# peach-xiao/EMRT

Hardware: AMD Instinct MI355X
Metric: training tiles/sec at 256x256 (higher is better)
Workload: dtype bf16; 1 GPU; EMRT ResNet50, Potsdam 256x256, 6 classes, batch 8 per GPU, fwd+bwd+SGD step (BASELINE configs[1]), bf16; global_batch=8, parallelism=dp1, hipgraph=True

## Files before the change

emrt_amd/csrc/common.hpp:

```cpp
#pragma once
#include <hip/hip_runtime.h>
#include <stdint.h>
#include <stdio.h>
#include <string.h>
#include "drop_hash.hpp"
#include "../../include/emrt_hip.h"

#define EMRT_F32 0
#define EMRT_BF16 1
#define EMRT_F16 2

namespace emrt {

extern thread_local char g_err[512];
inline int fail(const char* fn, const char* msg) {
  snprintf(g_err, sizeof(g_err), "%s: %s", fn, msg);
  return -1;
}
inline int check_launch(const char* fn) {
  hipError_t e = hipGetLastError();
  if (e != hipSuccess) {
    snprintf(g_err, sizeof(g_err), "%s: launch failed: %s", fn, hipGetErrorString(e));
    return -2;
  }
// ... 10 lines not shown
  int thin_cblk;
  int thin_blocks;
  int thin_ch;
  int no_thin_bwd;
  int igemm64_nst;
  int wgrad_nst;
  int pair_max;
  int msda_fwd_global;
  int msda_bwd_global;
  int msda_lds_min_pairs;
  int msda_bwd_dref_lds;
  int msda_band_halo;
  int msda_scatter_qsplit;
  int msda_scatter_cuts;
  int msda_fwd_chunks;
  int msda_fwd_threads;
  int msda_fwd_probe;
  int bn_block_kb;
  int bn_slice_c;
  int bn_operand_blocks;
  int ln_bwd_rows;
  int ln_bwd_max_blocks;
  int ln_bwd_threads;
  int ln_atomic;
  int gn_group_blocks;
  int gn_stat_rows;
  int gn_bwd_stat_rows;
  int gn_apply_rows;
  int igemm8p_probe;
  int igemm8p_cmajor;
  int igemm8p_min_blocks;
  int wgrad8p_min_steps;
  int wgrad8p_slab;
  int wgrad8p_xcd;
  int wgrad8p_force;
  int no_ksplit128;
  int wgrad_no_overwrite;
  int no_s2_dgrad;
  int wgroup_blocks;
  int wgroup_min_steps;
  int wgroup_max;
  int wgroup8;
  int wgroup8_blocks;
  int wgroup8_min_work;
  int msda_scatter_merge;
  int msda_scatter_mfma;
  int msda_mf_bands;
  int sgd_nt;
  int mha_bwd_split;
  int mha_valu;
  int no_bna;
  int memcpy_kernel;
  int xk;
};
extern Tuning g_tune;

struct Scratch {
  void* ptr; size_t bytes; void* stream;
  unsigned* tick;
  float* xk_part;
};
constexpr size_t SCRATCH_TICK_BYTES = 65536;
constexpr int SCRATCH_TICKS = (int)(SCRATCH_TICK_BYTES / 4);
constexpr size_t SCRATCH_XK_BYTES = 8u << 20;
extern Scratch g_scratch;

struct bf16_t {
  unsigned short v;
};
struct f16_t {
  unsigned short v;
};

__device__ __forceinline__ float to_f32(float x) { return x; }
__device__ __forceinline__ float to_f32(bf16_t x) { return __uint_as_float(((uint32_t)x.v) << 16); }
__device__ __forceinline__ float to_f32(f16_t x) { return (float)__builtin_bit_cast(_Float16, x.v); }
__device__ __forceinline__ float bf16_bits_to_f32(uint32_t lo16) { return __uint_as_float(lo16 << 16); }
__device__ __forceinline__ float f16_bits_to_f32(uint32_t lo16) { return (float)__builtin_bit_cast(_Float16, (unsigned short)lo16); }

template <class T>
__device__ __forceinline__ T from_f32(float f);
template <>
__device__ __forceinline__ float from_f32<float>(float f) {
  return f;
}
template <>
__device__ __forceinline__ bf16_t from_f32<bf16_t>(float f) {
  __bf16 b = (__bf16)f;
  bf16_t r;
  r.v = __builtin_bit_cast(unsigned short, b);
  return r;
}
template <>
__device__ __forceinline__ f16_t from_f32<f16_t>(float f) {
  f16_t r;
  r.v = __builtin_bit_cast(unsigned short, (_Float16)f);
  return r;
}
typedef __attribute__((ext_vector_type(2))) _Float16 emrt_half2_t;
typedef __attribute__((ext_vector_type(2))) float emrt_float2_t;
__device__ __forceinline__ uint32_t pack_f16x2(float lo, float hi) {
  emrt_half2_t h = __builtin_convertvector((emrt_float2_t){lo, hi}, emrt_half2_t);
  return __builtin_bit_cast(uint32_t, h);
}
__device__ __forceinline__ void unpack_f16x2(uint32_t w, float& lo, float& hi) {
  const emrt_half2_t h = __builtin_bit_cast(emrt_half2_t, w);
// ... 223 lines not shown
```

emrt_amd/csrc/conv.hip:

```cpp
#include "common.hpp"
#include "bn_operand.hpp"
#include <stdlib.h>
#include <type_traits>

using namespace emrt;

typedef __attribute__((ext_vector_type(8))) __bf16 bf16x8_t;
typedef __attribute__((ext_vector_type(4))) short short4_t;
typedef __attribute__((ext_vector_type(16))) float f32x16_t;

struct ConvArgs {
  const void* in = nullptr;
  const void* w = nullptr;
  void* out = nullptr;
  const float* bias = nullptr;
  const float* scale = nullptr;
  const void* res = nullptr;
  int N = 0, H = 0, W = 0, C = 0, ldin = 0;
  long long in_bs = 0;
  int OH = 0, OW = 0, OC = 0, ldout = 0;
  long long out_bs = 0;
  int ldres = 0;
  long long res_bs = 0;
  int KH = 0, KW = 0, stride = 0, pad = 0;
// ... 617 lines not shown
    }
  }
  if (p.stats) {
#pragma unroll
    for (int j = 0; j < TN; ++j) {
      const float s2 = st_s[j] + __shfl_xor(st_s[j], 32, 64);
      const float q2 = st_q[j] + __shfl_xor(st_q[j], 32, 64);
      const int n = bn * BN + (wc * TN + j) * 32 + frow;
      if (fh == 0 && n < p.OC) {
        double* rep = p.stats + (long long)(bm & 7) * 2 * p.OC;
        atomicAdd(rep + n, (double)s2);
        atomicAdd(rep + p.OC + n, (double)q2);
      }
    }
  }
}

template <class T, int TM, int TN, int WR, int WC, int MODE, bool VEC, int NST, int G>
__global__ __launch_bounds__(256 * G, (TM * TN == 1 && G == 1) ? 4 : 1) void igemm_kernel(ConvArgs p) {
  extern __shared__ __attribute__((aligned(16))) unsigned char smem_all[];
  igemm_body<T, TM, TN, WR, WC, MODE, VEC, NST, G>(p, (int)blockIdx.x, (int)gridDim.x, smem_all);
}

template <class T, int MODE>
__global__ __launch_bounds__(256, 4) void igemm_xk_kernel(ConvArgs p) {
  extern __shared__ __attribute__((aligned(16))) unsigned char smem_all[];
  igemm_body<T, 1, 1, 2, 2, MODE, true, 3, 1, false, true>(p, (int)blockIdx.x, (int)gridDim.x, smem_all);
}

template <class T>
__global__ __launch_bounds__(256, 4) void igemm_drop_kernel(ConvArgs p) {
  extern __shared__ __attribute__((aligned(16))) unsigned char smem_all[];
  igemm_body<T, 1, 1, 2, 2, 0, true, 3, 1, false, false, true>(p, (int)blockIdx.x, (int)gridDim.x, smem_all);
}

template <class T>
__global__ __launch_bounds__(256, 4) void igemm_s2_kernel(ConvArgs p) {
  extern __shared__ __attribute__((aligned(16))) unsigned char smem_all[];
  igemm_body<T, 1, 1, 2, 2, 1, true, 3, 1, true>(p, (int)blockIdx.x, (int)gridDim.x, smem_all);
}

template <class T, int G>
__global__ __launch_bounds__(256 * G, G == 1 ? 4 : 1) void igemm_bna_kernel(ConvArgs p) {
  extern __shared__ __attribute__((aligned(16))) unsigned char smem_all[];
  igemm_body<T, 1, 1, 2, 2, 0, true, (G == 2 ? 6 : 2), G, false, false, false, true>(p, (int)blockIdx.x, (int)gridDim.x, smem_all);
}
template <class T>
__global__ __launch_bounds__(256, 4) void igemm_xk_bna_kernel(ConvArgs p) {
  extern __shared__ __attribute__((aligned(16))) unsigned char smem_all[];
  igemm_body<T, 1, 1, 2, 2, 0, true, 2, 1, false, true, false, true>(p, (int)blockIdx.x, (int)gridDim.x, smem_all);
}

#include "igemm8p.hpp"

struct WgradArgs {
  const void* x = nullptr;
  const void* dy = nullptr;
  float* dw = nullptr;
  int N = 0, H = 0, W = 0, C = 0, ldx = 0;
  long long x_bs = 0;
  int OH = 0, OW = 0, OC = 0, lddy = 0;
  long long dy_bs = 0;
  int KH = 0, KW = 0, stride = 0, pad = 0;
  int dil = 1;
  int tiles_per_split = 0;
  float* dbias = nullptr;
  int overwrite = 0;
};

template <class T>
struct WgradCfg;
template <>
struct WgradCfg<bf16_t> {
  static constexpr int CPR = 16, RPP = 16, BKM = 64, PITCH = 320;
};
template <>
struct WgradCfg<float> {
  static constexpr int CPR = 32, RPP = 8, BKM = 32, PITCH = 528;
};

template <class T, bool VEC, int G, int NSTW = 2>
__device__ __forceinline__ void wgrad_body(const WgradArgs& p, const int block_x, const int block_y, const int block_z, unsigned char* smem_all) {
  using Cfg = WgradCfg<T>;
  constexpr int EPC = 16 / (int)sizeof(T);
  constexpr int CPR = Cfg::CPR, RPP = Cfg::RPP, BKM = Cfg::BKM, PITCH = Cfg::PITCH;
  constexpr int NST = VEC ? NSTW : 1;
  constexpr int STAGE_BYTES = 2 * BKM * PITCH;

  const int grp = G == 1 ? 0 : (int)threadIdx.x >> 8;
  unsigned char* smem = smem_all + grp * 2 * STAGE_BYTES;
  const int tid = threadIdx.x & 255, lane = tid & 63, wave = tid >> 6;
  const int wr = wave >> 1, wc = wave & 1;
  const int K = p.KH * p.KW * p.C;
  const int oc0 = block_y * 128, k0 = block_x * 128;
  const __amdgpu_buffer_rsrc_t rs_x = __builtin_amdgcn_make_buffer_rsrc((void*)p.x, 0, (int)BUF_RANGE, 0x00020000);
  const __amdgpu_buffer_rsrc_t rs_dy = __builtin_amdgcn_make_buffer_rsrc((void*)p.dy, 0, (int)BUF_RANGE, 0x00020000);

  const int col = tid % CPR, prow = tid / CPR;
  const int kq = k0 + col * EPC;
  const int tap = kq < K ? kq / p.C : 0;
  const int cq = kq - tap * p.C;
  const int kh = tap / p.KW, kw = tap - kh * p.KW;
  const int ocp = oc0 + col * EPC;
  const unsigned q_bad = kq < K ? 0u : BUF_OOB;
  const unsigned p_bad = ocp < p.OC ? 0u : BUF_OOB;
  int e_c[EPC], e_kh[EPC], e_kw[EPC];
// ... 305 lines not shown
  constexpr int BK = 8 * (16 / (int)sizeof(T));
  return (a.KH * a.KW * a.C + BK - 1) / BK;
}

template <class T>
static bool igemm_s2_ok(const ConvArgs& a) {
  constexpr int EPC = 16 / (int)sizeof(T);
  constexpr int BK = 8 * EPC;
  const long long M = (long long)a.N * a.OH * a.OW;
  if (a.KH * a.KW == 1 && g_tune.no_s2_dgrad != -1) return false;
  if (g_tune.no_s2_dgrad == 1 || a.stride != 2 || a.dil != 1 || a.C % BK != 0 || (a.OH & 1) || (a.OW & 1) || (M % 4) || ((M / 4) % 64) || a.OC <= 32 || a.OC % 8) return false;
  if (a.out_f32 || a.bias || a.scale) return false;
  auto al = [](const void* q) { return ((uintptr_t)q) % 16 == 0; };
  if (!al(a.out) || (a.res && !al(a.res)) || (a.mask_y && !al(a.mask_y)) || (a.stat_x && !al(a.stat_x))) return false;
  if (a.ldout % EPC || a.out_bs % EPC || (a.res && (a.ldres % EPC || a.res_bs % EPC)) || (a.mask_y && (a.ldy % EPC || a.y_bs % EPC)) ||
      (a.stat_x && (a.ldsx % EPC || a.sx_bs % EPC))) return false;
  return true;
}

template <class T>
static int igemm_xk_copies(const ConvArgs& a, hipStream_t st, int want) {
  constexpr int EPC = 16 / (int)sizeof(T);
  if (sizeof(T) != 2 || g_tune.xk < 0 || !g_scratch.xk_part || !g_scratch.tick || g_scratch.stream != (void*)st) return 0;
  if (a.OC <= 32 || a.OC % 8 || a.out_f32) return 0;
  auto al = [](const void* q) { return ((uintptr_t)q) % 16 == 0; };
  if (!al(a.out) || (a.res && !al(a.res)) || (a.mask_y && !al(a.mask_y)) || (a.stat_x && !al(a.stat_x))) return 0;
  if (a.ldout % EPC || a.out_bs % EPC || (a.res && (a.ldres % EPC || a.res_bs % EPC)) || (a.mask_y && (a.ldy % EPC || a.y_bs % EPC)) ||
      (a.stat_x && (a.ldsx % EPC || a.sx_bs % EPC))) return 0;
  const long long nb = conv_blocks(a, 64, 64);
  const int nkt = conv_k_tiles<T>(a);
  int S = want;
  if (S <= 0) {
    if (!((nb <= 64 && nkt >= 36) || (nb <= 128 && nkt >= 128))) return 0;
    S = 4;
  }
  if (S > nkt) S = nkt;
  if (S >= 2) {
    const int per = (nkt + S - 1) / S;
    S = (nkt + per - 1) / per;
  }
  if (S < 2 || nb > SCRATCH_TICKS || (size_t)nb * (size_t)S * 64 * 64 * 4 > SCRATCH_XK_BYTES) return 0;
  return S;
}

template <class T, int MODE>
static int launch_igemm_xk(const ConvArgs& a0, hipStream_t st, int S) {
  ConvArgs a = a0;
  const long long nb = conv_blocks(a, 64, 64);
  a.xk_S = S; a.xk_part = g_scratch.xk_part; a.xk_tick = g_scratch.tick;
  hipLaunchKernelGGL((igemm_xk_kernel<T, MODE>), dim3((unsigned)(nb * S)), dim3(256), (size_t)2 * 128 * 144, st, a);
  return check_launch("emrt_conv2d");
}


template <class T>
static bool conv_takes_128(const ConvArgs& a) {
  return a.OC > 64 && conv_k_tiles<T>(a) >= 16 && conv_blocks(a, 128, 128) >= 256;
}

enum ConvKind {
  CONV_NONE,
  CONV_DROP,
  CONV_S2,
  CONV_128x64,
  CONV_256x32,
  CONV_XK,
  CONV_8P,
  CONV_128,
  CONV_64
};
struct ConvPlan {
  ConvKind kind;
  int n;
  bool forced;
};

template <class T, int MODE, bool VEC>
static ConvPlan conv_plan(const ConvArgs& a, hipStream_t st) {
  constexpr bool VEC2 = VEC && sizeof(T) == 2;
  if (a.drop_seed) {
    constexpr int EPC = 16 / (int)sizeof(T);
    const bool vec_out = ((uintptr_t)a.out) % 16 == 0 && a.ldout % EPC == 0 && a.out_bs % EPC == 0 && a.OC % 8 == 0 && !a.out_f32 && !a.res && !a.mask_y;
    return {MODE == 0 && VEC && vec_out ? CONV_DROP : CONV_NONE, 1, false};
  }
  if (MODE == 1 && VEC && !g_tune.conv_tile && igemm_s2_ok<T>(a)) return {CONV_S2, 1, false};
  switch (g_tune.conv_tile) {
    case 1: return {CONV_64, 1, true};
    case 2: return {CONV_128x64, 1, true};
    case 3: return {CONV_128, 1, true};
    case 4: return {CONV_256x32, 1, true};
    case 5: if (VEC) return {CONV_64, 2, true}; break;
    case 6: if (VEC) return {CONV_64, 4, true}; break;
    case 7: if (VEC2 && igemm8p_ok<T>(a)) return {CONV_8P, 1, true}; break;
    case 8: if (VEC2) return {CONV_128, 2, true}; break;
    default: break;
  }
  if (a.OC <= 32) return {CONV_256x32, 1, false};
  if (VEC2 && !g_tune.conv_tile) {
    const int S = igemm_xk_copies<T>(a, st, g_tune.xk > 0 ? g_tune.xk : 0);
    if (S >= 2) return {CONV_XK, S, false};
  }
  if (VEC2) {
    const long long nb256 = conv_blocks(a, 256, 256);
    const int nkt64 = a.KH * a.KW * a.C / 64;
    const int minb = g_tune.igemm8p_min_blocks;
    if (minb > 0 && nkt64 >= 16 && (nb256 >= minb || (nb256 >= (minb * 3) / 5 && nkt64 >= 144)) && igemm8p_ok<T>(a)) return {CONV_8P, 1, false};
  }
  const int nkt = conv_k_tiles<T>(a);
  if (conv_takes_128<T>(a)) {
    const bool ksplit = VEC2 && nkt >= 32 && conv_blocks(a, 128, 128) == 256 && !g_tune.no_ksplit128;
    return {CONV_128, ksplit ? 2 : 1, false};
  }
  if (VEC) {
    const long long nb = conv_blocks(a, 64, 64);
    if (nb <= 128 && nkt >= 32) return {CONV_64, 4, false};
    if (nb <= 256 && nkt >= 16) return {CONV_64, 2, false};
  }
  return {CONV_64, 1, false};
}

template <class T, int MODE, bool VEC>
static int conv_launch(const ConvArgs& a, hipStream_t st, const ConvPlan& p) {
  constexpr bool VEC2 = VEC && sizeof(T) == 2;
  switch (p.kind) {
    case CONV_DROP:
      if constexpr (MODE == 0 && VEC) {
        hipLaunchKernelGGL((igemm_drop_kernel<T>), dim3((unsigned)conv_blocks(a, 64, 64)), dim3(256), (size_t)2 * 128 * 144, st, a);
        return check_launch("emrt_conv2d_drop");
      }
      break;
    case CONV_S2:
      if constexpr (MODE == 1 && VEC) {
        hipLaunchKernelGGL((igemm_s2_kernel<T>), dim3((unsigned)conv_blocks(a, 64, 64)), dim3(256), (size_t)2 * 128 * 144, st, a);
        return check_launch("emrt_conv2d");
      }
      break;
    case CONV_128x64: return launch_igemm<T, 2, 1, 2, 2, MODE, VEC>(a, st);
    case CONV_256x32: return launch_igemm<T, 2, 1, 4, 1, MODE, VEC>(a, st);
    case CONV_XK:
      if constexpr (VEC2) return launch_igemm_xk<T, MODE>(a, st, p.n);
      break;
    case CONV_8P:
      if constexpr (VEC2) return launch_igemm8p<T, MODE>(a, st);
      break;
    case CONV_128:
      if constexpr (VEC2) {
        if (p.n == 2) return launch_igemm<T, 2, 2, 2, 2, MODE, VEC, 2>(a, st);
      }
      return launch_igemm<T, 2, 2, 2, 2, MODE, VEC>(a, st);
    case CONV_64:
      if constexpr (VEC) {
        if (p.n == 4) return launch_igemm<T, 1, 1, 2, 2, MODE, VEC, 4>(a, st);
        if (p.n == 2) return launch_igemm<T, 1, 1, 2, 2, MODE, VEC, 2>(a, st);
      }
      return launch_igemm<T, 1, 1, 2, 2, MODE, VEC>(a, st);
    case CONV_NONE: break;
  }
  return fail("emrt_conv2d_drop", "needs 16-byte aligned rows of C, OC multiples of 8 elements (the vector path)");
}

template <class T, int MODE>
static int conv_dispatch(const ConvArgs& a, hipStream_t st) {
  if (conv_is_vec<T>(a)) return conv_launch<T, MODE, true>(a, st, conv_plan<T, MODE, true>(a, st));
  return conv_launch<T, MODE, false>(a, st, conv_plan<T, MODE, false>(a, st));
}

static ConvArgs conv_fwd_args(const void* in, const void* w_packed, void* out, const float* bias, const void* residual, int N, int H, int W, int C, int ldin,
                              long long in_bs, int OH, int OW, int OC, int ldout, long long out_bs, int ldres, long long res_bs, int KH, int KW, int stride,
                              int pad, int dilation, int relu, int out_f32, double* bn_stats, int cmajor, const float* out_scale) {
  ConvArgs a;
  a.in = in; a.w = w_packed; a.out = out; a.bias = bias; a.scale = out_scale; a.res = residual;
  a.N = N; a.H = H; a.W = W; a.C = C; a.ldin = ldin; a.in_bs = in_bs;
  a.OH = OH; a.OW = OW; a.OC = OC; a.ldout = ldout; a.out_bs = out_bs;
  a.ldres = ldres; a.res_bs = res_bs;
  a.KH = KH; a.KW = KW; a.stride = stride; a.pad = pad; a.dil = dilation; a.relu = relu; a.out_f32 = out_f32; a.cmajor = cmajor; a.stats = bn_stats;
  return a;
}

static ConvArgs conv_dgrad_args(const void* dy, const void* w_bwd_packed, void* dx, int lddx, long long dx_bs, int accumulate, const void* addend, int ldadd,
                                long long add_bs, int N, int H, int W, int C, int OH, int OW, int OC, int lddy, long long dy_bs, int KH, int KW, int stride,
                                int pad, int dilation, int cmajor, double* bn_stats = nullptr, const void* mask_y = nullptr, int ldy = 0, long long y_bs = 0,
                                float mask_scale = 1.f, const void* stat_x = nullptr, int ldsx = 0, long long sx_bs = 0) {
  ConvArgs d;
  d.in = dy; d.w = w_bwd_packed; d.out = dx;
  d.N = N; d.H = OH; d.W = OW; d.C = OC; d.ldin = lddy; d.in_bs = dy_bs;
  d.OH = H; d.OW = W; d.OC = C; d.ldout = lddx; d.out_bs = dx_bs;
  if (accumulate) { d.res = dx; d.ldres = lddx; d.res_bs = dx_bs; }
  else if (addend) { d.res = addend; d.ldres = ldadd; d.res_bs = add_bs; }
  d.KH = KH; d.KW = KW; d.stride = stride; d.pad = pad; d.dil = dilation; d.cmajor = cmajor; d.stats = bn_stats;
  d.mask_y = mask_y; d.ldy = ldy; d.y_bs = y_bs; d.mask_scale = mask_scale; d.stat_x = stat_x; d.ldsx = ldsx; d.sx_bs = sx_bs;
  return d;
}

static WgradArgs wgrad_args(const void* x, const void* dy, float* dw, float* dbias, int N, int H, int W, int C, int ldx, long long x_bs, int OH, int OW, int OC,
                            int lddy, long long dy_bs, int KH, int KW, int stride, int pad, int dilation, int overwrite) {
  WgradArgs a;
  a.x = x; a.dy = dy; a.dw = dw; a.dbias = dbias;
  a.N = N; a.H = H; a.W = W; a.C = C; a.ldx = ldx; a.x_bs = x_bs;
  a.OH = OH; a.OW = OW; a.OC = OC; a.lddy = lddy; a.dy_bs = dy_bs;
  a.KH = KH; a.KW = KW; a.stride = stride; a.pad = pad; a.dil = dilation; a.overwrite = overwrite;
  return a;
}

struct ConvShape { int N, H, W, C, OH, OW, OC, KH, KW, stride, pad, dil; };
enum {
  CK_DIMS = 1, CK_KERNEL = 2, CK_SIZE = 4, CK_PIXELS = 8,
  CK_X = 16, CK_Y = 32, CK_W = 64,
  CK_X24 = 128, CK_Y24 = 256,
// ... 37 lines not shown
                       int dilation, const float* out_scale, float drop_p, const unsigned long long* drop_seed, unsigned drop_salt, int dtype, void* stream) {
  EMRT_REQUIRE(in && w_packed && out, "null pointer");
  const ConvShape s = mode == 1 ? ConvShape{N, OH, OW, OC, H, W, C, KH, KW, stride, pad, dilation} : ConvShape{N, H, W, C, OH, OW, OC, KH, KW, stride, pad, dilation};
  EMRT_CONV_CHECK(s, 0, 0, 0, 0, dtype, CK_DIMS | CK_KERNEL);
  EMRT_REQUIRE(mode == 0 || mode == 1, "mode must be 0 (fwd) or 1 (dgrad)");
  EMRT_CONV_CHECK(s, 0, 0, 0, 0, dtype, CK_PIXELS);
  EMRT_REQUIRE_FWD_DTYPE(dtype);
  EMRT_REQUIRE(dtype != EMRT_F16 || mode == 0, "fp16 (dtype 2) is inference-only: forward convolution (mode 0)");
  EMRT_REQUIRE(conv_size_ok(s), mode == 0 ? "fwd: output size mismatch" : "dgrad: size mismatch");
  EMRT_CONV_CHECK(s, ldin, in_bs, ldin, in_bs, dtype, (mode == 0 ? CK_X : CK_Y) | CK_W);
  ConvArgs a = conv_fwd_args(in, w_packed, out, bias, residual, N, H, W, C, ldin, in_bs, OH, OW, OC, ldout, out_bs, ldres, res_bs, KH, KW, stride, pad, dilation,
                             relu, out_f32, bn_stats, g_tune.igemm8p_cmajor, out_scale);
  a.mask_y = mask_y; a.ldy = ldy; a.y_bs = y_bs;
  if (drop_p > 0.f) { a.drop_seed = drop_seed; a.drop_salt = drop_salt; a.drop_p = drop_p; }
  EMRT_REQUIRE(!mask_y || !out_f32, "the ReLU mask needs an output in the compute dtype");
  hipStream_t st = (hipStream_t)stream;
  return with_fwd_dtype(__func__, dtype, [&](auto t) {
    using T = decltype(t);
    if constexpr (std::is_same<T, f16_t>::value) return conv_dispatch<T, 0>(a, st);
    else return mode == 0 ? conv_dispatch<T, 0>(a, st) : conv_dispatch<T, 1>(a, st);
  });
}

extern "C" int emrt_conv2d(const void* in, const void* w_packed, void* out, const float* bias, const void* residual,
                           int N, int H, int W, int C, int ldin, long long in_bs,
                           int OH, int OW, int OC, int ldout, long long out_bs,
                           int ldres, long long res_bs,
                           int KH, int KW, int stride, int pad,
                           int mode, int relu, int out_f32, double* bn_stats, const void* mask_y, int ldy, long long y_bs,
                           int dilation, const float* out_scale, int dtype, void* stream) {
  return conv2d_impl(in, w_packed, out, bias, residual, N, H, W, C, ldin, in_bs, OH, OW, OC, ldout, out_bs, ldres, res_bs, KH, KW, stride, pad,
                     mode, relu, out_f32, bn_stats, mask_y, ldy, y_bs, dilation, out_scale, 0.f, nullptr, 0u, dtype, stream);
}

extern "C" int emrt_conv2d_drop(const void* in, const void* w_packed, void* out, const float* bias, int M, int C, int ldin, int OC, int ldout,
                                float p, const unsigned long long* seed, unsigned salt, int dtype, void* stream) {
  EMRT_REQUIRE_TRAIN_DTYPE(dtype);
  EMRT_REQUIRE(seed && p > 0.f && p < 1.f, "needs a device seed and 0 < p < 1");
  EMRT_REQUIRE(M > 0 && C > 0 && OC > 0 && OC % 8 == 0 && (long long)M * OC < (1ll << 32), "bad dims (OC a multiple of 8, fewer than 2^32 outputs)");
  return conv2d_impl(in, w_packed, out, bias, nullptr, 1, 1, M, C, ldin, (long long)M * ldin, 1, M, OC, ldout, (long long)M * ldout, 0, 0, 1, 1, 1, 0,
                     0, 1, 0, nullptr, nullptr, 0, 0, 1, nullptr, p, seed, salt, dtype, stream);
}

template <class T>
static ConvPlan bna_plan(const ConvArgs& a, hipStream_t st) {
  constexpr int BK = 8 * (16 / (int)sizeof(T));
  const ConvPlan none = {CONV_NONE, 0, false};
  if (!conv_is_vec<T>(a) || a.C % BK != 0 || a.C > 1024 || a.OC <= 32) return none;
  if (a.stride != 1 || a.KH != a.KW || (a.KH != 1 && a.KH != 3) || a.pad != a.dil * (a.KH >> 1) || a.OH != a.H || a.OW != a.W) return none;
  if (((uintptr_t)a.a_out) % 16 != 0) return none;
  if (a.KH == 3 && a.C > 128 && g_tune.no_bna != -1) return none;
  const ConvPlan p = conv_plan<T, 0, true>(a, st);
  if (g_tune.conv_tile && !p.forced) return none;
  return p.kind == CONV_64 || p.kind == CONV_XK ? p : none;
}

template <class T>
static int launch_bna(const ConvArgs& a0, hipStream_t st, const ConvPlan& p) {
  ConvArgs a = a0;
  const long long nb = conv_blocks(a, 64, 64);
  const size_t tab = (size_t)2 * a.C * sizeof(float);
  if (p.kind == CONV_XK) {
    a.xk_S = p.n; a.xk_part = g_scratch.xk_part; a.xk_tick = g_scratch.tick;
    hipLaunchKernelGGL((igemm_xk_bna_kernel<T>), dim3((unsigned)(nb * a.xk_S)), dim3(256), (size_t)2 * 128 * 144 + tab, st, a);
    return check_launch("emrt_conv2d_bna");
  }
  const int G = p.n;
  size_t lds = (size_t)G * 2 * 128 * 144 + tab;
  if (G > 1 && lds < (size_t)(G - 1) * 16 * 256 * 4) lds = (size_t)(G - 1) * 16 * 256 * 4;
  static bool attr_done = false;
  if (!attr_done) {
    if (hipFuncSetAttribute(reinterpret_cast<const void*>(igemm_bna_kernel<T, 2>), hipFuncAttributeMaxDynamicSharedMemorySize, 160 * 1024) != hipSuccess ||
        hipFuncSetAttribute(reinterpret_cast<const void*>(igemm_bna_kernel<T, 4>), hipFuncAttributeMaxDynamicSharedMemorySize, 160 * 1024) != hipSuccess)
      return fail("emrt_conv2d_bna", "cannot raise the dynamic LDS limit");
    attr_done = true;
  }
  if (G == 1) hipLaunchKernelGGL((igemm_bna_kernel<T, 1>), dim3((unsigned)nb), dim3(256), lds, st, a);
  else if (G == 2) hipLaunchKernelGGL((igemm_bna_kernel<T, 2>), dim3((unsigned)nb), dim3(512), lds, st, a);
  else hipLaunchKernelGGL((igemm_bna_kernel<T, 4>), dim3((unsigned)nb), dim3(1024), lds, st, a);
  return check_launch("emrt_conv2d_bna");
}

static ConvArgs bna_args(const void* in, const void* w_packed, void* out, const float* bias, const void* residual, int N, int H, int W, int C, int ldin,
                         long long in_bs, int OH, int OW, int OC, int ldout, long long out_bs, int ldres, long long res_bs, int KH, int KW, int stride, int pad,
                         int relu, int out_f32, double* bn_stats, int dilation, const double* sums, double count, float eps, float momentum, float* mean,
                         float* invstd, float* run_mean, float* run_var, const float* gamma, const float* beta, int in_relu, void* a_out) {
  ConvArgs a = conv_fwd_args(in, w_packed, out, bias, residual, N, H, W, C, ldin, in_bs, OH, OW, OC, ldout, out_bs, ldres, res_bs, KH, KW, stride, pad, dilation,
                             relu, out_f32, bn_stats, 0, nullptr);
  a.bna.sums = sums; a.bna.inv_count = count > 0.0 ? 1.0 / count : 0.0; a.bna.eps = eps; a.bna.momentum = momentum; a.bna.mean = mean; a.bna.invstd = invstd;
  a.bna.run_mean = run_mean; a.bna.run_var = run_var; a.bna.gamma = gamma; a.bna.beta = beta; a.bna.relu = in_relu;
  a.a_out = a_out;
  return a;
}

extern "C" int emrt_conv2d_bna_supported(const void* in, const void* w_packed, void* out, const float* bias, const void* residual, int N, int H, int W, int C,
                                         int ldin, long long in_bs, int OH, int OW, int OC, int ldout, long long out_bs, int ldres, long long res_bs, int KH,
                                         int KW, int stride, int pad, int relu, int out_f32, double* bn_stats, int dilation, const double* sums, double count,
                                         float eps, float momentum, float* mean, float* invstd, float* run_mean, float* run_var, const float* gamma,
                                         const float* beta, int in_relu, void* a_out, int dtype, void* stream) {
  if (!(dtype == EMRT_F32 || dtype == EMRT_BF16) || !in || !w_packed || !out || !sums || !mean || !invstd || !gamma || !beta || !a_out || count <= 0.0) return 0;
  if (N <= 0 || H <= 0 || W <= 0 || C <= 0 || OC <= 0 || dilation < 1 || g_tune.no_bna == 1) return 0;
  const long long esz = dtype == EMRT_F32 ? 4 : 2;
  if ((long long)N * H * W * C * esz >= (1ll << 31) || (long long)N * H * W + 512 >= (1ll << 31)) return 0;
  if (((long long)(N - 1) * in_bs + ((long long)H * W - 1) * ldin + C) * esz >= (1ll << 31) || (long long)OC * KH * KW * C * esz >= (1ll << 31)) return 0;
  const ConvArgs a = bna_args(in, w_packed, out, bias, residual, N, H, W, C, ldin, in_bs, OH, OW, OC, ldout, out_bs, ldres, res_bs, KH, KW, stride, pad, relu, out_f32,
                              bn_stats, dilation, sums, count, eps, momentum, mean, invstd, run_mean, run_var, gamma, beta, in_relu, a_out);
  hipStream_t st = (hipStream_t)stream;
  return with_train_dtype("emrt_conv2d_bna_supported", dtype, [&](auto t) { return bna_plan<decltype(t)>(a, st).kind != CONV_NONE ? 1 : 0; });
}

extern "C" int emrt_conv2d_bna(const void* in, const void* w_packed, void* out, const float* bias, const void* residual, int N, int H, int W, int C,
                               int ldin, long long in_bs, int OH, int OW, int OC, int ldout, long long out_bs, int ldres, long long res_bs, int KH,
                               int KW, int stride, int pad, int relu, int out_f32, double* bn_stats, int dilation, const double* sums, double count,
                               float eps, float momentum, float* mean, float* invstd, float* run_mean, float* run_var, const float* gamma,
// ... 896 lines not shown
```

emrt_amd/csrc/elementwise.hip:

```cpp
#include "common.hpp"
#include <stdlib.h>

using namespace emrt;

thread_local char emrt::g_err[512] = {0};

extern "C" const char* emrt_last_error(void) { return emrt::g_err; }
extern "C" int emrt_abi_version(void) { return 9; }

namespace {
struct TuneEntry { const char* name; int emrt::Tuning::*field; int def; };
const TuneEntry kTune[] = {
    {"conv_tile", &emrt::Tuning::conv_tile, 0},         {"wgrad_split", &emrt::Tuning::wgrad_split, 0},
    {"thin_cblk", &emrt::Tuning::thin_cblk, 64},        {"thin_blocks", &emrt::Tuning::thin_blocks, 128},
    {"thin_ch", &emrt::Tuning::thin_ch, 8},             {"no_thin_bwd", &emrt::Tuning::no_thin_bwd, 0},
    {"pair_max", &emrt::Tuning::pair_max, 768},         {"msda_fwd_global", &emrt::Tuning::msda_fwd_global, 0},
    {"bn_block_kb", &emrt::Tuning::bn_block_kb, 0},     {"ln_atomic", &emrt::Tuning::ln_atomic, 1},
    {"bn_slice_c", &emrt::Tuning::bn_slice_c, 0},
    {"msda_fwd_chunks", &emrt::Tuning::msda_fwd_chunks, 0}, {"msda_fwd_threads", &emrt::Tuning::msda_fwd_threads, 1024},
    {"msda_fwd_probe", &emrt::Tuning::msda_fwd_probe, 0}, {"wgrad_nst", &emrt::Tuning::wgrad_nst, 2},
    {"igemm64_nst", &emrt::Tuning::igemm64_nst, 3}, {"msda_bwd_global", &emrt::Tuning::msda_bwd_global, 0},
    {"msda_lds_min_pairs", &emrt::Tuning::msda_lds_min_pairs, 2048}, {"msda_bwd_dref_lds", &emrt::Tuning::msda_bwd_dref_lds, 1},
    {"gn_group_blocks", &emrt::Tuning::gn_group_blocks, 0}, {"gn_stat_rows", &emrt::Tuning::gn_stat_rows, 32},
    {"gn_bwd_stat_rows", &emrt::Tuning::gn_bwd_stat_rows, 32}, {"gn_apply_rows", &emrt::Tuning::gn_apply_rows, 8},
    {"msda_scatter_cuts", &emrt::Tuning::msda_scatter_cuts, 0}, {"msda_scatter_qsplit", &emrt::Tuning::msda_scatter_qsplit, 0}, {"msda_band_halo", &emrt::Tuning::msda_band_halo, 0},
    {"igemm8p_probe", &emrt::Tuning::igemm8p_probe, 0}, {"igemm8p_min_blocks", &emrt::Tuning::igemm8p_min_blocks, 160}, {"igemm8p_cmajor", &emrt::Tuning::igemm8p_cmajor, 0},
    {"wgrad8p_min_steps", &emrt::Tuning::wgrad8p_min_steps, 8}, {"wgrad8p_slab", &emrt::Tuning::wgrad8p_slab, 1}, {"wgrad8p_force", &emrt::Tuning::wgrad8p_force, 0}, {"wgrad8p_xcd", &emrt::Tuning::wgrad8p_xcd, 1},
    {"wgrad_no_overwrite", &emrt::Tuning::wgrad_no_overwrite, 0}, {"no_ksplit128", &emrt::Tuning::no_ksplit128, 0}, {"ln_bwd_rows", &emrt::Tuning::ln_bwd_rows, 0}, {"ln_bwd_max_blocks", &emrt::Tuning::ln_bwd_max_blocks, 0}, {"bn_operand_blocks", &emrt::Tuning::bn_operand_blocks, 0}, {"no_s2_dgrad", &emrt::Tuning::no_s2_dgrad, 0}, {"wgroup_blocks", &emrt::Tuning::wgroup_blocks, 1024}, {"wgroup_min_steps", &emrt::Tuning::wgroup_min_steps, 32}, {"wgroup_max", &emrt::Tuning::wgroup_max, 0},
    {"no_bna", &emrt::Tuning::no_bna, 0}, {"memcpy_kernel", &emrt::Tuning::memcpy_kernel, 0}, {"xk", &emrt::Tuning::xk, 0}, {"mha_valu", &emrt::Tuning::mha_valu, 0}, {"mha_bwd_split", &emrt::Tuning::mha_bwd_split, 1}, {"msda_scatter_merge", &emrt::Tuning::msda_scatter_merge, 0},
    {"wgroup8", &emrt::Tuning::wgroup8, 0}, {"wgroup8_blocks", &emrt::Tuning::wgroup8_blocks, 0}, {"wgroup8_min_work", &emrt::Tuning::wgroup8_min_work, 6000},
    {"msda_scatter_mfma", &emrt::Tuning::msda_scatter_mfma, 1}, {"sgd_nt", &emrt::Tuning::sgd_nt, 1}, {"ln_bwd_threads", &emrt::Tuning::ln_bwd_threads, 512}, {"msda_mf_bands", &emrt::Tuning::msda_mf_bands, 0},
};
emrt::Tuning tuning_from_env() {
  emrt::Tuning t;
  for (const TuneEntry& e : kTune) {
    char env[64] = "EMRT_";
    size_t n = strlen(env);
    for (const char* c = e.name; *c && n + 1 < sizeof(env); ++c) env[n++] = (char)((*c >= 'a' && *c <= 'z') ? *c - 32 : *c);
    env[n] = 0;
    const char* v = (strcmp(e.name, "msda_fwd_probe") == 0 || strcmp(e.name, "igemm8p_probe") == 0) ? nullptr : getenv(env);
    t.*(e.field) = v ? atoi(v) : e.def;
  }
  return t;
}
}
emrt::Tuning emrt::g_tune = tuning_from_env();
emrt::Scratch emrt::g_scratch = {nullptr, 0, nullptr, nullptr, nullptr};

extern "C" int emrt_set_scratch(void* ptr, size_t bytes, void* stream) {
  EMRT_REQUIRE((ptr != nullptr) == (bytes > 0) && ((uintptr_t)ptr) % 256 == 0, "scratch must be 256-byte aligned device memory (or nullptr, 0)");
  if (ptr && ptr == emrt::g_scratch.ptr && emrt::g_scratch.tick && bytes == emrt::g_scratch.bytes + emrt::SCRATCH_TICK_BYTES + emrt::SCRATCH_XK_BYTES) {
    emrt::g_scratch.stream = stream;
    return 0;
  }
  emrt::g_scratch.ptr = ptr;
  emrt::g_scratch.bytes = bytes;
  emrt::g_scratch.stream = stream;
  emrt::g_scratch.tick = nullptr;
  emrt::g_scratch.xk_part = nullptr;
  if (ptr && bytes >= (16u << 20) + emrt::SCRATCH_XK_BYTES + emrt::SCRATCH_TICK_BYTES && bytes % 256 == 0) {
    emrt::g_scratch.bytes = bytes - emrt::SCRATCH_TICK_BYTES - emrt::SCRATCH_XK_BYTES;
    emrt::g_scratch.xk_part = reinterpret_cast<float*>(static_cast<char*>(ptr) + emrt::g_scratch.bytes);
    emrt::g_scratch.tick = reinterpret_cast<unsigned*>(static_cast<char*>(ptr) + emrt::g_scratch.bytes + emrt::SCRATCH_XK_BYTES);
    if (hipMemsetAsync(emrt::g_scratch.tick, 0, emrt::SCRATCH_TICK_BYTES, (hipStream_t)stream) != hipSuccess) {
      emrt::g_scratch.tick = nullptr;
      return emrt::fail("emrt_set_scratch", "cannot zero the arrival counters");
    }
  }
  return 0;
}

extern "C" int emrt_set_tuning(const char* name, int value) {
  EMRT_REQUIRE(name, "null name");
  for (const TuneEntry& e : kTune)
    if (strcmp(e.name, name) == 0) { emrt::g_tune.*(e.field) = value; return 0; }
  return emrt::fail("emrt_set_tuning", "unknown knob");
}
extern "C" int emrt_get_tuning(const char* name, int* value) {
  EMRT_REQUIRE(name && value, "null pointer");
  for (const TuneEntry& e : kTune)
    if (strcmp(e.name, name) == 0) { *value = emrt::g_tune.*(e.field); return 0; }
  return emrt::fail("emrt_get_tuning", "unknown knob");
}

// ... 398 lines not shown
```

Measured before the change: 1044 tiles/s.

## Add row-panel kernel for 1x1 convs with small K reusing A tile across output chunks

Adds a specialized pointwise-conv kernel for 1x1 stride-1 convs with C<=128 and OC>=128. Each block loads its 64-row A tile once into registers, keeps it resident, and walks a panel of 64-wide output chunks, streaming weights with prefetch. It fuses the existing epilogue: bias/scale, residual, relu, mask, BN stats, and an optional BN-apply prologue. The aim is to cut redundant A reads and launch-tile overhead for the many ResNet bottleneck expand convs. It adds code complexity and a per-chunk syncthreads cost, and it changes which kernels serve these layers.

New measurement: 1047 tiles/s (median of 6 runs). About the same (+0.3%).

```diff
diff --git a/emrt_amd/csrc/common.hpp b/emrt_amd/csrc/common.hpp
--- a/emrt_amd/csrc/common.hpp
+++ b/emrt_amd/csrc/common.hpp
@@ -86,6 +86,9 @@
   int no_bna;
   int memcpy_kernel;
   int xk;
+  int pw_rows;
+  int pw_panel;
+  int pw_rows_count;
 };
 extern Tuning g_tune;
 
diff --git a/emrt_amd/csrc/conv.hip b/emrt_amd/csrc/conv.hip
--- a/emrt_amd/csrc/conv.hip
+++ b/emrt_amd/csrc/conv.hip
@@ -693,6 +693,7 @@
 }
 
 #include "igemm8p.hpp"
+#include "pw_rows.hpp"
 
 struct WgradArgs {
   const void* x = nullptr;
@@ -1104,6 +1105,47 @@
   return check_launch("emrt_conv2d");
 }
 
+constexpr long long PW_MIN_ROWS = 8192;
+template <class T>
+static int pw_rows_panel(const ConvArgs& a) {
+  constexpr int EPC = 16 / (int)sizeof(T);
+  if (sizeof(T) != 2 || g_tune.pw_rows < 0 || g_tune.conv_tile) return 0;
+  if (g_tune.pw_rows > 0 && g_tune.pw_rows != 64) return 0;
+  if (a.KH != 1 || a.KW != 1 || a.stride != 1 || a.pad != 0 || a.OH != a.H || a.OW != a.W || a.C > 128 || a.OC < 128 || a.OC % 8 || a.drop_seed) return 0;
+  auto al = [](const void* q) { return ((uintptr_t)q) % 16 == 0; };
+  if (!al(a.out) || (a.res && !al(a.res)) || (a.mask_y && !al(a.mask_y)) || (a.stat_x && !al(a.stat_x))) return 0;
+  const int eo = a.out_f32 ? 4 : EPC;
+  if (a.ldout % eo || a.out_bs % eo || (a.res && (a.ldres % EPC || a.res_bs % EPC)) || (a.mask_y && (a.ldy % EPC || a.y_bs % EPC)) ||
+      (a.stat_x && (a.ldsx % EPC || a.sx_bs % EPC))) return 0;
+  const long long M = (long long)a.N * a.OH * a.OW;
+  if (g_tune.pw_rows == 0 && M < PW_MIN_ROWS) return 0;
+  const long long tiles_m = (M + 63) / 64;
+  const int nchunks = (a.OC + 63) / 64;
+  if (g_tune.pw_panel > 0) {
+    const int pc = (g_tune.pw_panel + 63) / 64;
+    return pc < nchunks ? pc : nchunks;
+  }
+  long long want = (512 + tiles_m - 1) / tiles_m;
+  if (want > nchunks) want = nchunks;
+  return (int)((nchunks + want - 1) / want);
+}
+
+template <class T, bool BNA>
+static int launch_pw_rows(const ConvArgs& a, hipStream_t st, int panel_chunks, const char* fn) {
+  if constexpr (sizeof(T) == 2) {
+    const long long M = (long long)a.N * a.OH * a.OW;
+    const int nchunks = (a.OC + 63) / 64;
+    const long long grid = ((M + 63) / 64) * ((nchunks + panel_chunks - 1) / panel_chunks);
+    const int nkt = (a.C + 63) / 64;
+    const size_t lds = (size_t)64 * 72 * 4 + (size_t)nkt * 64 * 144 + (BNA ? (size_t)2 * a.C * sizeof(float) : 0);
+    if (nkt == 1) hipLaunchKernelGGL((pw_rows_kernel<T, 1, BNA>), dim3((unsigned)grid), dim3(256), lds, st, a, panel_chunks);
+    else hipLaunchKernelGGL((pw_rows_kernel<T, 2, BNA>), dim3((unsigned)grid), dim3(256), lds, st, a, panel_chunks);
+    ++g_tune.pw_rows_count;
+    return check_launch(fn);
+  }
+  return fail(fn, "the row-panel kernel is built for 2-byte element types");
+}
+
 
 template <class T>
 static bool conv_takes_128(const ConvArgs& a) {
@@ -1119,7 +1161,8 @@
   CONV_XK,
   CONV_8P,
   CONV_128,
-  CONV_64
+  CONV_64,
+  CONV_PW
 };
 struct ConvPlan {
   ConvKind kind;
@@ -1167,6 +1210,10 @@
     const long long nb = conv_blocks(a, 64, 64);
     if (nb <= 128 && nkt >= 32) return {CONV_64, 4, false};
     if (nb <= 256 && nkt >= 16) return {CONV_64, 2, false};
+    if constexpr (VEC2) {
+      const int pc = pw_rows_panel<T>(a);
+      if (pc > 0) return {CONV_PW, pc, false};
+    }
   }
   return {CONV_64, 1, false};
 }
@@ -1206,6 +1253,9 @@
         if (p.n == 2) return launch_igemm<T, 1, 1, 2, 2, MODE, VEC, 2>(a, st);
       }
       return launch_igemm<T, 1, 1, 2, 2, MODE, VEC>(a, st);
+    case CONV_PW:
+      if constexpr (VEC2) return launch_pw_rows<T, false>(a, st, p.n, "emrt_conv2d");
+      break;
     case CONV_NONE: break;
   }
   return fail("emrt_conv2d_drop", "needs 16-byte aligned rows of C, OC multiples of 8 elements (the vector path)");
@@ -1349,7 +1399,7 @@
   if (a.KH == 3 && a.C > 128 && g_tune.no_bna != -1) return none;
   const ConvPlan p = conv_plan<T, 0, true>(a, st);
   if (g_tune.conv_tile && !p.forced) return none;
-  return p.kind == CONV_64 || p.kind == CONV_XK ? p : none;
+  return p.kind == CONV_64 || p.kind == CONV_XK || p.kind == CONV_PW ? p : none;
 }
 
 template <class T>
@@ -1357,6 +1407,7 @@
   ConvArgs a = a0;
   const long long nb = conv_blocks(a, 64, 64);
   const size_t tab = (size_t)2 * a.C * sizeof(float);
+  if (p.kind == CONV_PW) return launch_pw_rows<T, true>(a, st, p.n, "emrt_conv2d_bna");
   if (p.kind == CONV_XK) {
     a.xk_S = p.n; a.xk_part = g_scratch.xk_part; a.xk_tick = g_scratch.tick;
     hipLaunchKernelGGL((igemm_xk_bna_kernel<T>), dim3((unsigned)(nb * a.xk_S)), dim3(256), (size_t)2 * 128 * 144 + tab, st, a);
diff --git a/emrt_amd/csrc/elementwise.hip b/emrt_amd/csrc/elementwise.hip
--- a/emrt_amd/csrc/elementwise.hip
+++ b/emrt_amd/csrc/elementwise.hip
@@ -30,6 +30,7 @@
     {"no_bna", &emrt::Tuning::no_bna, 0}, {"memcpy_kernel", &emrt::Tuning::memcpy_kernel, 0}, {"xk", &emrt::Tuning::xk, 0}, {"mha_valu", &emrt::Tuning::mha_valu, 0}, {"mha_bwd_split", &emrt::Tuning::mha_bwd_split, 1}, {"msda_scatter_merge", &emrt::Tuning::msda_scatter_merge, 0},
     {"wgroup8", &emrt::Tuning::wgroup8, 0}, {"wgroup8_blocks", &emrt::Tuning::wgroup8_blocks, 0}, {"wgroup8_min_work", &emrt::Tuning::wgroup8_min_work, 6000},
     {"msda_scatter_mfma", &emrt::Tuning::msda_scatter_mfma, 1}, {"sgd_nt", &emrt::Tuning::sgd_nt, 1}, {"ln_bwd_threads", &emrt::Tuning::ln_bwd_threads, 512}, {"msda_mf_bands", &emrt::Tuning::msda_mf_bands, 0},
+    {"pw_rows", &emrt::Tuning::pw_rows, 0}, {"pw_panel", &emrt::Tuning::pw_panel, 0}, {"pw_rows_count", &emrt::Tuning::pw_rows_count, 0},
 };
 emrt::Tuning tuning_from_env() {
   emrt::Tuning t;
diff --git a/emrt_amd/csrc/pw_rows.hpp b/emrt_amd/csrc/pw_rows.hpp
--- /dev/null
+++ b/emrt_amd/csrc/pw_rows.hpp
@@ -0,0 +1,249 @@
+#pragma once
+
+template <class T>
+__device__ __forceinline__ uint32_t pw_bna_word2(uint32_t w, const float2 s2, const float2 h2, bool do_relu) {
+  typedef float f32x2_t __attribute__((ext_vector_type(2)));
+  typedef __bf16 bf16x2_t __attribute__((ext_vector_type(2)));
+  typedef short i16x2_t __attribute__((ext_vector_type(2)));
+  if constexpr (std::is_same<T, bf16_t>::value) {
+    const f32x2_t e = {__uint_as_float(w << 16), __uint_as_float(w & 0xffff0000u)};
+    const f32x2_t r = __builtin_elementwise_fma(e, f32x2_t{s2.x, s2.y}, f32x2_t{h2.x, h2.y});
+    const bf16x2_t b = __builtin_convertvector(r, bf16x2_t);
+    i16x2_t bi = __builtin_bit_cast(i16x2_t, b);
+    if (do_relu) bi = __builtin_elementwise_max(bi, i16x2_t{0, 0});
+    return __builtin_bit_cast(uint32_t, bi);
+  } else {
+    const float lo = do_relu ? 0.f : -INFINITY;
+    float e0, e1;
+    unpack_f16x2(w, e0, e1);
+    e0 = fmaxf(fmaf(e0, s2.x, h2.x), lo);
+    e1 = fmaxf(fmaf(e1, s2.y, h2.y), lo);
+    return pack_f16x2(e0, e1);
+  }
+}
+
+template <class T, int NKT, bool BNA>
+__global__ __launch_bounds__(256, 2) void pw_rows_kernel(ConvArgs p, int panel_chunks) {
+  static_assert(sizeof(T) == 2 && (NKT == 1 || NKT == 2), "2-byte elements, K <= 128");
+  constexpr int BM = 64, BN = 64, EPC = 8, BK = 64, PITCH = 144;
+  constexpr int CP = BN + 8, CGR = BN / 8, RP = 256 / CGR, RPT = BM / RP;
+  extern __shared__ __attribute__((aligned(16))) unsigned char smem_all[];
+  constexpr int A_BYTES = NKT * BM * PITCH > BM * CP * 4 ? NKT * BM * PITCH : BM * CP * 4;
+  unsigned char* sA = smem_all;
+  float* tile = reinterpret_cast<float*>(smem_all);
+  unsigned char* sB = smem_all + A_BYTES;
+  float* bn_tab = reinterpret_cast<float*>(sB + NKT * BN * PITCH);
+
+  const int tid = (int)threadIdx.x, lane = tid & 63, wave = tid >> 6;
+  const int wr = wave >> 1, wc = wave & 1;
+  const int frow = lane & 31, fh = lane >> 5;
+  const int chunk = tid & 7, row0 = tid >> 3;
+  const int K = p.C;
+  const int nchunks = (p.OC + BN - 1) / BN;
+  const int panels = (nchunks + panel_chunks - 1) / panel_chunks;
+  int bid = (int)blockIdx.x;
+  const int nblk = (int)gridDim.x;
+  if ((nblk & 7) == 0) bid = (bid & 7) * (nblk >> 3) + (bid >> 3);
+  const int bm = bid / panels, pn = bid - bm * panels;
+  const int gc0 = pn * panel_chunks;
+  const int nch = nchunks - gc0 < panel_chunks ? nchunks - gc0 : panel_chunks;
+  const int OHW = p.OH * p.OW;
+  const long long M = (long long)p.N * OHW;
+
+  const __amdgpu_buffer_rsrc_t rs_in = __builtin_amdgcn_make_buffer_rsrc((void*)p.in, 0, (int)BUF_RANGE, 0x00020000);
+  const __amdgpu_buffer_rsrc_t rs_w = __builtin_amdgcn_make_buffer_rsrc((void*)p.w, 0, (int)BUF_RANGE, 0x00020000);
+
+  uint4 ra[NKT][2], rb[NKT][2];
+  bool a_ok[2];
+  unsigned a_m[2];
+#pragma unroll
+  for (int i = 0; i < 2; ++i) {
+    const unsigned m = (unsigned)bm * (unsigned)BM + (unsigned)(row0 + 32 * i);
+    a_ok[i] = (long long)m < M;
+    a_m[i] = m;
+    const unsigned mm = a_ok[i] ? m : 0u;
+    const int nb = (int)(mm / (unsigned)OHW);
+    const int pix = (int)(mm - (unsigned)nb * (unsigned)OHW);
+    const unsigned off = (unsigned)((long long)nb * p.in_bs * (long long)sizeof(T)) + (unsigned)(pix * p.ldin) * (unsigned)sizeof(T);
+    const unsigned a_off = a_ok[i] ? off : BUF_OOB;
+#pragma unroll
+    for (int kt = 0; kt < NKT; ++kt) {
+      const int k0 = kt * BK + chunk * EPC;
+      const unsigned kbad = k0 < K ? 0u : BUF_OOB;
+      ra[kt][i] = buf_load16(rs_in, (a_off | kbad) + (unsigned)k0 * (unsigned)sizeof(T));
+    }
+  }
+  auto load_b = [&](int gc, bool live) {
+#pragma unroll
+    for (int j = 0; j < 2; ++j) {
+      const int n = gc * BN + row0 + 32 * j;
+      const unsigned b_off = (live && n < p.OC) ? (unsigned)((long long)n * K * (long long)sizeof(T)) : BUF_OOB;
+#pragma unroll
+      for (int kt = 0; kt < NKT; ++kt) {
+        const int k0 = kt * BK + chunk * EPC;
+        const unsigned kbad = k0 < K ? 0u : BUF_OOB;
+        rb[kt][j] = buf_load16(rs_w, (b_off | kbad) + (unsigned)k0 * (unsigned)sizeof(T));
+      }
+    }
+  };
+  auto store_b = [&]() {
+#pragma unroll
+    for (int kt = 0; kt < NKT; ++kt)
+#pragma unroll
+      for (int j = 0; j < 2; ++j) *reinterpret_cast<uint4*>(sB + (kt * BN + row0 + 32 * j) * PITCH + chunk * 16) = rb[kt][j];
+  };
+  load_b(gc0, true);
+
+  if constexpr (BNA) {
+    bn_operand_preamble(p.bna, p.C, bn_tab, blockIdx.x == 0);
+    const __amdgpu_buffer_rsrc_t rs_aout = __builtin_amdgcn_make_buffer_rsrc(p.a_out, 0, (int)BUF_RANGE, 0x00020000);
+    const bool do_relu = p.bna.relu != 0;
+#pragma unroll
+    for (int kt = 0; kt < NKT; ++kt) {
+      const int c0 = kt * BK + chunk * EPC;
+      const float* tsc = bn_tab + c0;
+      const float* tsh = bn_tab + p.C + c0;
+      uint32_t wq[2][4];
+#pragma unroll
+      for (int i = 0; i < 2; ++i) { wq[i][0] = ra[kt][i].x; wq[i][1] = ra[kt][i].y; wq[i][2] = ra[kt][i].z; wq[i][3] = ra[kt][i].w; }
+#pragma unroll
+      for (int q = 0; q < 4; ++q) {
+        const float2 s2 = *reinterpret_cast<const float2*>(tsc + 2 * q), h2 = *reinterpret_cast<const float2*>(tsh + 2 * q);
+#pragma unroll
+        for (int i = 0; i < 2; ++i) wq[i][q] = a_ok[i] ? pw_bna_word2<T>(wq[i][q], s2, h2, do_relu) : 0u;
+      }
+#pragma unroll
+      for (int i = 0; i < 2; ++i) {
+        ra[kt][i] = make_uint4(wq[i][0], wq[i][1], wq[i][2], wq[i][3]);
+        const unsigned wb = (pn == 0 && a_ok[i]) ? a_m[i] * (unsigned)p.C * (unsigned)sizeof(T) : BUF_OOB;
+        __builtin_amdgcn_raw_buffer_store_b128(u32x4_t{ra[kt][i].x, ra[kt][i].y, ra[kt][i].z, ra[kt][i].w}, rs_aout, (int)(wb + (unsigned)c0 * (unsigned)sizeof(T)), 0, 0);
+      }
+    }
+  }
+#pragma unroll
+  for (int kt = 0; kt < NKT; ++kt)
+#pragma unroll
+    for (int i = 0; i < 2; ++i) *reinterpret_cast<uint4*>(sA + (kt * BM + row0 + 32 * i) * PITCH + chunk * 16) = ra[kt][i];
+  store_b();
+  __syncthreads();
+  uint4 fa[NKT][4];
+#pragma unroll
+  for (int kt = 0; kt < NKT; ++kt)
+#pragma unroll
+    for (int s = 0; s < 4; ++s) fa[kt][s] = *reinterpret_cast<const uint4*>(sA + (kt * BM + wr * 32 + frow) * PITCH + (2 * s + fh) * 16);
+  __syncthreads();
+
+  const int cg = tid % CGR, rr = tid / CGR;
+  bool r_ok[RPT];
+  int e_nb[RPT], e_pix[RPT];
+#pragma unroll
+  for (int r = 0; r < RPT; ++r) {
+    const unsigned m = (unsigned)bm * (unsigned)BM + (unsigned)(rr + r * RP);
+    r_ok[r] = (long long)m < M;
+    const unsigned mm = r_ok[r] ? m : 0u;
+    e_nb[r] = (int)(mm / (unsigned)OHW);
+    e_pix[r] = (int)(mm - (unsigned)e_nb[r] * (unsigned)OHW);
+  }
+  const T* resp = (const T*)p.res;
+  const T* ymask = (const T*)p.mask_y;
+  const T* sxp = (const T*)p.stat_x;
+
+  for (int j = 0; j < nch; ++j) {
+    const int gc = gc0 + j;
+    load_b(gc + 1, j + 1 < nch);
+    const int n0 = gc * BN + cg * 8;
+    const bool col_ok = n0 < p.OC;
+    float bv[8], sv[8];
+#pragma unroll
+    for (int e = 0; e < 8; ++e) { bv[e] = (p.bias && col_ok) ? p.bias[n0 + e] : 0.f; sv[e] = (p.scale && col_ok) ? p.scale[n0 + e] : 1.f; }
+    uint4 q_res[RPT], q_msk[RPT], q_sx[RPT];
+#pragma unroll
+    for (int r = 0; r < RPT; ++r) {
+      q_res[r] = q_msk[r] = q_sx[r] = make_uint4(0u, 0u, 0u, 0u);
+      if (r_ok[r] && col_ok) {
+        if (resp) q_res[r] = *reinterpret_cast<const uint4*>(resp + (long long)e_nb[r] * p.res_bs + (long long)e_pix[r] * p.ldres + n0);
+        if (ymask) {
+          q_msk[r] = *reinterpret_cast<const uint4*>(ymask + (long long)e_nb[r] * p.y_bs + (long long)e_pix[r] * p.ldy + n0);
+          if (sxp) q_sx[r] = *reinterpret_cast<const uint4*>(sxp + (long long)e_nb[r] * p.sx_bs + (long long)e_pix[r] * p.ldsx + n0);
+        }
+      }
+    }
+
+    f32x16_t acc;
+#pragma unroll
+    for (int r = 0; r < 16; ++r) acc[r] = 0.f;
+#pragma unroll
+    for (int kt = 0; kt < NKT; ++kt)
+#pragma unroll
+      for (int s = 0; s < 4; ++s) {
+        const uint4 fb = *reinterpret_cast<const uint4*>(sB + (kt * BN + wc * 32 + frow) * PITCH + (2 * s + fh) * 16);
+        mma_chunk<T>(acc, fa[kt][s], fb);
+      }
+#pragma unroll
+    for (int r = 0; r < 16; ++r) tile[(wr * 32 + (r & 3) + 8 * (r >> 2) + 4 * fh) * CP + wc * 32 + frow] = acc[r];
+    __syncthreads();
+
+    float ss[8], sq[8];
+#pragma unroll
+    for (int e = 0; e < 8; ++e) { ss[e] = 0.f; sq[e] = 0.f; }
+#pragma unroll
+    for (int r = 0; r < RPT; ++r) {
+      if (!r_ok[r] || !col_ok) continue;
+      const int row = rr + r * RP;
+      const float4 a = *reinterpret_cast<const float4*>(tile + row * CP + cg * 8);
+      const float4 b = *reinterpret_cast<const float4*>(tile + row * CP + cg * 8 + 4);
+      float v[8] = {a.x, a.y, a.z, a.w, b.x, b.y, b.z, b.w};
+#pragma unroll
+      for (int e = 0; e < 8; ++e) v[e] = fmaf(v[e], sv[e], bv[e]);
+      if (resp) {
+        float w8[8];
+        Vec8<T>::unpack(q_res[r], w8);
+#pragma unroll
+        for (int e = 0; e < 8; ++e) v[e] += w8[e];
+      }
+      if (p.relu) {
+#pragma unroll
+        for (int e = 0; e < 8; ++e) v[e] = fmaxf(v[e], 0.f);
+      }
+      float second[8];
+      if (ymask) {
+        Vec8<T>::unpack(q_msk[r], second);
+#pragma unroll
+        for (int e = 0; e < 8; ++e) v[e] = second[e] > 0.f ? v[e] * p.mask_scale : 0.f;
+        if (sxp) Vec8<T>::unpack(q_sx[r], second);
+      }
+      const long long obase = (long long)e_nb[r] * p.out_bs + (long long)e_pix[r] * p.ldout + n0;
+      if (p.out_f32) {
+        Vec8<float>::store((float*)p.out + obase, v);
+      } else {
+        Vec8<T>::store((T*)p.out + obase, v);
+#pragma unroll
+        for (int e = 0; e < 8; ++e) v[e] = to_f32(from_f32<T>(v[e]));
+      }
+#pragma unroll
+      for (int e = 0; e < 8; ++e) {
+        ss[e] += v[e];
+        sq[e] = fmaf(v[e], ymask ? second[e] : v[e], sq[e]);
+      }
+    }
+    store_b();
+    if (p.stats) {
+      __syncthreads();
+      float* red = tile;
+#pragma unroll
+      for (int e = 0; e < 8; ++e) {
+        red[rr * BN + cg * 8 + e] = ss[e];
+        red[(RP + rr) * BN + cg * 8 + e] = sq[e];
+      }
+      __syncthreads();
+      if (tid < 2 * BN) {
+        const int which = tid / BN, col = tid % BN;
+        const int n = gc * BN + col;
+        float a = 0.f;
+        for (int q = 0; q < RP; ++q) a += red[(which * RP + q) * BN + col];
+        if (n < p.OC) atomicAdd(p.stats + (long long)(bm & 7) * 2 * p.OC + (long long)which * p.OC + n, (double)a);
+      }
+    }
+    __syncthreads();
+  }
+}
```
